# richardshuai/ExPecto

Hardware: AMD Instinct MI355X
Metric: variants/sec (200 windows × 2002 feats) at 1/2/4/8 MI355X; HBM GB/s vs peak (higher is better)
Workload: dtype fp32 in/out (f16x3: power-of-2-scaled 2-way fp16 split = 22-bit operands, 3 MFMA products, fp32 accumulate; bf16x6 recompute on fp16 overflow)

## Files before the change

### expecto_amd/csrc/beluga.hip

```cpp
#include <hip/hip_runtime.h>

#include <algorithm>
#include <array>
#include <cstdint>
#include <cstdlib>
#include <cstring>
#include <map>
#include <memory>
#include <mutex>
#include <tuple>
#include <string>
#include <vector>

#include "beluga_knobs.h"
#include "common.h"
#include "event_pairs.h"
#include "gemm_kernel.h"
#include "seg_plan.h"

namespace expecto {

static_assert(kStrandFwd == EXPECTO_STRAND_FWD && kStrandRc == EXPECTO_STRAND_RC && kStrandBoth == EXPECTO_STRAND_BOTH &&
              EXPECTO_EINVAL == -1, "seg_plan.h restates the strand modes and the refusal code");
constexpr int kNFeat = 2002;
// ... 475 lines not shown

__global__ __launch_bounds__(64) void slab_macs(const unsigned* __restrict__ mask, int tiles, double per_bit,
                                                double* __restrict__ acc) {
  int bits = 0;
  for (int i = threadIdx.x; i < tiles; i += 64) bits += __popc(mask[i]);
  for (int o = 32; o > 0; o >>= 1) bits += __shfl_down(bits, o);
  if (threadIdx.x == 0) atomicAdd(acc, bits * per_bit);
}

__global__ __launch_bounds__(256) void pair_patch_apply(const float* __restrict__ d6, float* __restrict__ act6, int nv,
                                                        int v0, const int* __restrict__ var_pos, int row16) {
  const int m = blockIdx.x;
  const int r6 = delta_rows(pair_pos(var_pos, m, nv, v0)).r[6];
  const floatx4* src = reinterpret_cast<const floatx4*>(d6) + (long long)m * kDW[6] * row16;
  floatx4* dst = reinterpret_cast<floatx4*>(act6) + ((long long)m * 106 + r6) * row16;
  for (int k = threadIdx.x; k < kDW[6] * row16; k += blockDim.x) dst[k] = src[k];
}

constexpr int kSegTab = 20;
constexpr int kW4u = 19, kA4u = 26;
struct SegDims {
  int L, T1, P1, T3, T4, S5, T5, T6;
};

__global__ void seg_delta_table(const int* __restrict__ var_pos, int e0, int ns, SegStrands ss, SegDims g, int n_ph,
                                int4 ph, int* __restrict__ tab) {
  const int m = blockIdx.x * blockDim.x + threadIdx.x;
  if (m >= ns) return;
  const int e = e0 + m;
  int q = min(max(var_pos[e >= ss.n_seg ? e - ss.n_seg : e], 0), g.L - 1);
  if (e >= ss.rc_ent) q = g.L - 1 - q;
  int* t = tab + m * kSegTab;
  const int r1 = clampi(q - 7, 0, g.T1 - kDW[1]);
  const int r2 = clampi(floor4(r1 - 7), 0, g.P1 - kDW[2]);
  const int r3 = clampi(r2 - 7, 0, g.T3 - kDW[3]);
  const int r4 = clampi(r3 - 7, 0, g.T4 - kW4u);
  t[0] = q;
  t[1] = r1;
  t[2] = r2;
  t[3] = r3;
  t[4] = r4;
  for (int i = 0; i < n_ph; ++i) {
    const int p = i == 0 ? ph.x : i == 1 ? ph.y : i == 2 ? ph.z : ph.w;
    const int r4p = clampi(floor4(r4 - p), 0, g.S5 - kDW[4]);
    const int r5 = clampi(r4p - 7, 0, g.T5 - kDW[5]);
    t[5 + i] = r4p;
// ... 163 lines not shown
  const int q = o >> 2, p = q & 3, off6 = (q - p) >> 2;
  const int pi = p == 0 ? ph_idx.x : p == 1 ? ph_idx.y : p == 2 ? ph_idx.z : ph_idx.w;
  const int r6 = tab[(win_seg[w] + sd * ss.n_seg - ent_base) * kSegTab + 13 + pi];
  const int lo = max(r6 - off6, 0), hi = min(r6 + kDW[6] - off6, 106);
  if (lo >= hi) return;
  unsigned bits = 0;
  for (int ks = lo * 640 / slab_k; ks <= (hi * 640 - 1) / slab_k; ++ks) bits |= 1u << ks;
  atomicOr(mask + m / tile_rows, bits);
}

__global__ void copy_rows(const float* __restrict__ src, float* __restrict__ dst, const int* __restrict__ widx,
                          const int* __restrict__ win_row, int n_win, long long rc_rows) {
  const int v = widx[blockIdx.x];
  const int sd = v >= n_win ? 1 : 0, w = v - sd * n_win;
  const long long r = (sd * rc_rows + (win_row ? win_row[w] : w)) * kNFeat;
  for (int i = threadIdx.x; i < kNFeat; i += blockDim.x) dst[r + i] = src[r + i];
}

__global__ void pair_rows(long long* __restrict__ c_rows, int M, int nv, int v0, long long strand_stride) {
  const int m = blockIdx.x * blockDim.x + threadIdx.x;
  if (m < M) c_rows[m] = (long long)(m / nv) * strand_stride + v0 + m % nv;
}

constexpr int kFkK = 16000;
constexpr int kFkKb = kFkK / GBK;
constexpr int kFkSlabs = 2;
constexpr int kFkTailK = kFc1In - 4 * kFkK;
constexpr int kFkKbTotal = 9 * kFkKb + kFkTailK / GBK;
constexpr long long kFkKTotal = 9LL * kFkK + kFkTailK;
constexpr int kFkSeq[9] = {3, 2, 3, 1, 0, 1, 3, 2, 3};
constexpr int kFkBlk[9] = {0, 1, 1, 2, 3, 3, 2, 3, 3};
constexpr int kFkRole[4][4] = {{0, 1, 3, 4}, {1, 2, 4, 5}, {3, 4, 6, 7}, {4, 5, 7, 8}};
constexpr int kFkW[9][4] = {{1, 0, 0, 0}, {1, 1, 0, 0}, {0, -1, 0, 0}, {1, 0, 1, 0}, {1, 1, 1, 1},
                            {0, -1, 0, -1}, {0, 0, -1, 0}, {0, 0, -1, -1}, {0, 0, 0, 1}};
constexpr int kFkParts = 4 * kFkSlabs + 1;

__global__ void fk_weights(const float* __restrict__ w1, long long rows, float* __restrict__ wk) {
  const long long i = (long long)blockIdx.x * blockDim.x + threadIdx.x;
  if (i >= rows * kFkKTotal) return;
  const long long n = i / kFkKTotal;
  const int k = (int)(i - n * kFkKTotal);
  const float* wr = w1 + n * kFc1In;
  if (k >= 9 * kFkK) {
    wk[i] = wr[4 * kFkK + (k - 9 * kFkK)];
    return;
  }
  const int g = k / kFkK, kk = k - g * kFkK;
  double s = 0.0;
#pragma unroll
  for (int q = 0; q < 4; ++q)
    if (kFkW[g][q]) s += kFkW[g][q] * (double)wr[q * kFkK + kk];
  wk[i] = (float)s;
}

__global__ __launch_bounds__(320) void fk_seq_h2(const float* __restrict__ x, int T, int s, const int* __restrict__ tab,
// ... 1306 lines not shown
    else
      fc2_reduce1<<<dim3((unsigned)(((long long)nb * kNFeat + 255) / 256)), dim3(256), 0, st>>>(
          h->part2, h->fc2_splits, (long long)nb * kHidLd, nb, h->fc2b, a.col_scale, c_rows, y);
    if ((rc = check_launch("fc2_reduce"))) return rc;
  }
  return EXPECTO_OK;
}

int run_fc(expecto_beluga* h, const float* act, const long long* a_rows, int nb, float* y, hipStream_t st,
           const long long* c_rows = nullptr, const unsigned* ks_mask = nullptr, double slab_frac = 1.0,
           long long part_rows = 0) {
  int rc;
  if ((rc = run_fc1(h, act, a_rows, nb, h->h1, st, ks_mask, slab_frac, part_rows))) return rc;
  return run_fc2(h, h->h1, nb, y, st, c_rows);
}

int count_desc_macs(expecto_beluga* h, const unsigned* mask, int tiles, double per_tile, hipStream_t st);

bool fk_use(const expecto_beluga* h) {
  return h->fk_on && h->fkw && g_precision == EXPECTO_PRECISION_F16X3 && h->fk_role < 4;
}
bool fk_use_seg(const expecto_beluga* h) { return h->fk_on && h->fkw && g_precision == EXPECTO_PRECISION_F16X3; }

int fk_cap(const expecto_beluga* h) { return std::max(h->max_batch, h->fk_slice); }
constexpr int kGresPerBatch = 3;

int fk_tables(expecto_beluga* h) {
  if (h->fk_grows) return EXPECTO_OK;
  const size_t mb = h->max_batch, tiles = (mb + 255) / 256, cap = fk_cap(h);
  float *a = nullptr, *b = nullptr, *c = nullptr, *d = nullptr;
  int rc;
  if ((rc = dalloc(h, &a, 2 * 9 * cap)) || (rc = dalloc(h, &b, 2 * mb)) || (rc = dalloc(h, &c, kFkParts * cap)) ||
      (rc = dalloc(h, &d, kFkParts * tiles)))
    return rc;
  h->fk_grows = reinterpret_cast<long long*>(a);
  h->fk_wrows = reinterpret_cast<long long*>(b);
  h->fk_prow = reinterpret_cast<int*>(c);
  h->fk_mask = reinterpret_cast<unsigned*>(d);
  return EXPECTO_OK;
}

int fk_seg_buffers(expecto_beluga* h) {
  if (h->fk_part) return EXPECTO_OK;
  const size_t cap = fk_cap(h);
  float *a = nullptr, *b = nullptr;
  int rc;
  if ((rc = dalloc(h, &h->fk_part, (size_t)kFkParts * cap * kHidLd)) || (rc = dalloc(h, &h->fk_h1, act_alloc(cap * kHidLd))) ||
// ... 20 lines not shown
    if ((rc = b.reserve(((size_t)rows + 16) * 640, h->bytes))) break;
  return rc;
}

int fk_sequences(expecto_beluga* h, const float* x, long long blocks, int T, int s, const int* tab, int n_ph,
                 hipStream_t st, const int* gres = nullptr, int set = 0) {
  int rc;
  if ((rc = fk_seq_alloc(h, blocks * s, set))) return rc;
  const DevBuf<float>* out = set ? h->fk_aseq : h->fk_seq;
  Timer lt(h, 7, st);
  const long long nblk = blocks * 7;
  EXPECTO_REQUIRE(nblk > 0 && nblk < (1LL << 31), "FC1 sequence grid");
  fk_seq_h2<<<dim3((unsigned)nblk), dim3(320), 0, st>>>(x, T, s, tab, n_ph, gres, out[0], out[1], out[2], h->ovf);
  return check_launch("fk_seq_h2");
}

struct FkProducts {
  const long long* g_rows;
  int off[9];
  int cnt[9];
  int lay[9];
};

int fk_reduce(expecto_beluga* h, const float* part, const int* prow, int n, float* h1, hipStream_t st) {
  Timer lt(h, 7, st);
  const long long count4 = (long long)n * (kHidLd / 4);
  fk_reduce_h2<<<dim3((unsigned)((count4 + 255) / 256)), dim3(256), 0, st>>>(part, prow, count4, h->fc1b, h1, h->fk_cs,
                                                                           exp2i(h->sx[6]), h->ovf);
  return check_launch("fk_reduce_h2");
}

constexpr int kFcNarrowNb = 7;
static_assert(kHidLd % (16 * kFcNarrowNb) == 0 && kHidLd % FCW_BN == 0, "FC1 N tiles");
bool fc1_narrow(const expecto_beluga* h, long long mtt) {
  if (h->fc1_narrow >= 0) return h->fc1_narrow != 0;
  if (!h->narrow_scope) return false;
  const long long cus = h->cus > 0 ? h->cus : 256;
  return mtt * (kHidLd / (16 * kFcNarrowNb)) <= cus;
}

static_assert(kHidLd % (16 * FCS_NB) == 0 &&
                  (kNFeat + 16 * FCS_NB - 1) / (16 * FCS_NB) * 16 * FCS_NB <= (kNFeat + GBN - 1) / GBN * GBN,
              "skinny FC tiles");
bool fc_skinny(const expecto_beluga* h, long long rows) {
  return h->fc_skinny && rows <= 32 && (h->fc1_narrow >= 0 ? h->fc1_narrow != 0 : h->narrow_scope);
}

int fk_fc1(expecto_beluga* h, const float* x, const DevBuf<float>* seq, const FkProducts& pr, const long long* w_rows, int n,
           const int* prow, float* h1, hipStream_t st, const unsigned* mask = nullptr, int tiles = 0,
           float* part = nullptr, long long part_cap = 0) {
  if (!part) {
    part = h->part;
    part_cap = (long long)std::max(h->fc_splits, kFkParts) * h->max_batch;
  }
  FcGroup G{};
  G.kb_total = kFkKbTotal;
  G.n_tiles = (kHidLd + FCW_BN - 1) / FCW_BN;
  G.n_store = kHidLd;
  G.ldc = kHidLd;
  const char* wb = reinterpret_cast<const char*>(h->fkw);
  long long row = 0;
  long long blk = 0;
  int mslot = 0;
  double macs = 0.0;
  auto add = [&](const float* A, const long long* ar, long long aoff, int kb0, int nk, int M, int lay) {
    FcDesc& d = G.d[G.n];
    d.A = A;
    d.a_rows = ar;
    d.a_off = aoff;
    d.Bp = wb + (long long)kb0 * 128;
    d.C = part + row * kHidLd;
    d.mask = mask ? mask + (size_t)mslot * tiles : nullptr;
    ++mslot;
    d.M = M;
    d.m_tiles = (M + X6P_BM - 1) / X6P_BM;
    d.nk = nk;
    d.blk0 = (int)blk;
    blk += (long long)d.m_tiles * G.n_tiles;
    row += lay;
    macs += (double)M * kFc1Out * nk * GBK;
    ++G.n;
  };
  for (int g = 0; g < 9; ++g) {
    const int lay = pr.lay[g] ? pr.lay[g] : pr.cnt[g];
    for (int s = 0; lay > 0 && s < kFkSlabs; ++s) {
      if (pr.cnt[g] > 0)
        add(kFkSeq[g] ? seq[kFkSeq[g] - 1].p : x, pr.g_rows + pr.off[g], 25LL * kFkBlk[g] * 640 + (long long)s * kFkK / kFkSlabs,
            g * kFkKb + s * kFkKb / kFkSlabs, kFkKb / kFkSlabs, pr.cnt[g], lay);
      else {
        row += lay;
        ++mslot;
      }
    }
  }
  add(x, w_rows, 100LL * 640, 9 * kFkKb, kFkTailK / GBK, n, n);
  EXPECTO_REQUIRE(G.n <= FCK_MAX && blk < (1LL << 31), "Karatsuba FC1 descriptors");
  EXPECTO_REQUIRE(row <= part_cap, "Karatsuba FC1 partial rows");
  {
    Timer lt(h, 6, st);
    if (h->profiling) {
      if (!mask) {
        h->macs[h->timer_base + 6] += macs;
      } else {
        for (int i = 0; i < G.n; ++i) {
          const FcDesc& d = G.d[i];
          int rc = count_desc_macs(h, d.mask, d.m_tiles, (double)d.M / d.m_tiles * kFc1Out * d.nk * GBK, st);
          if (rc) return rc;
        }
      }
    }
    G.rr = mask ? 0 : 1;
    const long long mtt = blk / G.n_tiles;
    const bool narrow = !mask && fc1_narrow(h, mtt);
    if (narrow) {
      G.n_tiles = kHidLd / (16 * kFcNarrowNb);
      for (int i = 0; i < G.n; ++i) G.d[i].blk0 = G.d[i].blk0 / (kHidLd / FCW_BN) * G.n_tiles;
    }
    const long long grid = G.rr ? (mtt + 7) / 8 * 8 * G.n_tiles : mtt * G.n_tiles;
    if (narrow)
      beluga_fc_h3k_narrow<<<dim3((unsigned)grid), dim3(512), 0, st>>>(G);
// ... 202 lines not shown
  return run_conv(c.h, l, c.h->DA, dnext, (long long)ck.ns * nbk, arows, w, w, pool, c.sa);
}
int seg_st_wait(const SegCall& c, hipEvent_t e) {
  if (c.sa != c.st) EXPECTO_HIP_CHECK(hipStreamWaitEvent(c.st, e, 0));
  return EXPECTO_OK;
}

int seg_rows(const SegCall& c, const SegChunk& ck, const int* widx, int w0, int n, long long* a_rows,
             long long* c_rows) {
  seg_a_rows<<<dim3((n + 255) / 256), dim3(256), 0, c.st>>>(c.h->win_seg_d, c.h->win_off_d, c.win_row_d, widx, w0, n,
                                                             ck.s0, c.pl.ss, c.pl.g.L, c.pl.n_ph, c.phi, c.pl.g.T6,
                                                             a_rows, c_rows);
  return check_launch("seg_a_rows");
}

int seg_fc2(const SegCall& c, const float* h1, int n, float* y, const long long* c_rows) {
  int rc;
  for (int r0 = 0; r0 < n; r0 += c.h->max_batch)
    if ((rc = run_fc2(c.h, h1 + (long long)r0 * kHidLd, std::min(c.h->max_batch, n - r0), y, c.st, c_rows + r0)))
      return rc;
  return EXPECTO_OK;
}

int seg_alt_conv6(const SegCall& c, const SegChunk& ck) {
  int rc;
  if ((rc = seg_st_wait(c, c.h->pev[13]))) return rc;
  seg_alt_blocks<<<dim3(kAltRows6, (unsigned)ck.nb), dim3(64), 0, c.st>>>(c.h->P, c.h->D0, c.pl.n_ph, c.pl.g.T6,
                                                                           c.h->seg_tab, 640 * c.eb / 16, c.h->Q);
  return check_launch("seg_alt_blocks");
}

int seg_copy_tail(const SegCall& c, const SegChunk& ck) {
  if (!c.pr) return EXPECTO_OK;
  const std::vector<int>& cw = c.pl.copy_w;
  const int ic0 = (int)(std::lower_bound(cw.begin(), cw.end(), ck.w0) - cw.begin());
  const int ic1 = (int)(std::lower_bound(cw.begin(), cw.end(), ck.w0 + ck.nw) - cw.begin());
  if (ic1 <= ic0) return EXPECTO_OK;
  copy_rows<<<dim3(ic1 - ic0), dim3(256), 0, c.st>>>(c.y, c.pr->y_alt, c.h->copy_w_d + ic0, c.win_row_d, c.pl.ss.n_win,
                                                      c.pl.ss.rc_rows);
  return check_launch("copy_rows");
}

int seg_trunk(const SegCall& c, const SegChunk& ck, PQSwap& pq) {
  expecto_beluga* h = c.h;
  const SegPairs* pr = c.pr;
  const SegGeo& g = c.pl.g;
  const hipStream_t st = c.st, sa = c.sa;
  const int s0 = ck.s0, ns = ck.ns, n_ph = c.pl.n_ph;
  const long long nb = ck.nb;
  int rc;
  if (pr && (rc = stream_order(st, sa, h->pev[0]))) return rc;
// ... 111 lines not shown
    t.pa.cnt[gq] = cnt;
    t.pa.lay[gq] = prd.cnt[gq];
    for (int sb = 0; prd.cnt[gq] > 0 && sb < kFkSlabs; ++sb) {
      t.md.g[t.md.n] = gq;
      t.md.s[t.md.n] = sb;
      t.md.off[t.md.n] = prd.off[gq];
      t.md.cnt[t.md.n] = cnt;
      ++t.md.n;
    }
  }
  t.md.nw = (int)sl.nw_pre;
  for (size_t i = 0; i < sl.nw_pre; ++i) {
    const FkWin& w = ws[sl.i0 + i];
    t.winfo.push_back(w.blk);
    t.winfo.push_back(w.off6);
    if (pl.v_is_alt(w.w)) {
      t.aperm.push_back(w.w);
      t.aprow.insert(t.aprow.end(), prow.begin() + (long long)i * kFkParts, prow.begin() + (long long)(i + 1) * kFkParts);
    }
  }
  return t;
}

int seg_fc_karatsuba(const SegCall& c, const SegChunk& ck) {
  expecto_beluga* h = c.h;
  const SegPlan& pl = c.pl;
  const hipStream_t st = c.st;
  const int T6 = pl.g.T6, n_ph = pl.n_ph;
  const long long nb = ck.nb, cap = pl.fk_cap;
  const std::vector<FkWin>& ws = pl.fk_ref[ck.ci];
  const int* perm = h->fc_perm_d + ck.w0;
  int rc;
  const std::vector<int> gres = pl.fk_gres(ck.ci);
  EXPECTO_REQUIRE(nb <= kGresPerBatch * (long long)h->max_batch, "conv6 blocks of a chunk exceed fk_gres");
  if ((rc = stage_copies(h, {{h->fk_gres, gres.data(), gres.size() * sizeof(int)}}, st)) || (rc = fk_tables(h)) ||
      (rc = fk_seg_buffers(h)) || (rc = fk_sequences(h, h->P, nb, T6, T6, nullptr, n_ph, st, h->fk_gres)))
    return rc;
  bool alt_ready = false;
  FkSlice sl{};
  for (size_t i0 = 0; i0 < ws.size(); i0 = sl.i1) {
    const char* refusal = pl.fk_slice(ck.ci, i0, sl);
    EXPECTO_REQUIRE(!refusal, refusal);
    const int fn = (int)(sl.i1 - i0);
    std::vector<long long> grows;
    std::vector<int> prow, rgrp, ginfo;
    FkProducts prd{h->fk_grows, {}, {}, {}};
    fk_slice_tables(ws, (int)i0, (int)sl.i1, T6, grows, prd, prow, &rgrp, &ginfo);
    if ((rc = stage_copies(h, {{h->fk_grows, grows.data(), grows.size() * sizeof(long long)},
                               {h->fk_prow, prow.data(), prow.size() * sizeof(int)}}, st)) ||
        (rc = seg_rows(c, ck, perm + i0, 0, fn, h->fk_arows, h->fk_crows)) ||
        (rc = fk_fc1(h, h->P, h->fk_seq, prd, h->fk_arows, fn, h->fk_prow, h->fk_h1, st, nullptr, 0, h->fk_part,
                     kFkParts * cap)) ||
        (rc = seg_fc2(c, h->fk_h1, fn, c.y, h->fk_crows)))
      return rc;
    if (sl.n_ag == 0) continue;
    const FkAltTables t = fk_alt_tables(pl, ws, sl, prd, rgrp, prow);
    const int na = (int)t.aperm.size();
    const int tiles = (int)(cap / 256 + 1);
    if ((rc = stage_copies(h, {{h->fk_rgrp, rgrp.data(), rgrp.size() * sizeof(int)},
                               {h->fk_ginfo, ginfo.data(), ginfo.size() * sizeof(int)},
                               {h->fk_winfo, t.winfo.data(), t.winfo.size() * sizeof(int)},
                               {h->fk_aperm, t.aperm.data(), t.aperm.size() * sizeof(int)},
                               {h->fk_aprow, t.aprow.data(), t.aprow.size() * sizeof(int)}}, st)))
      return rc;
    if (!alt_ready) {
      if ((rc = seg_alt_conv6(c, ck))) return rc;
      DeltaScope ds(h);
      if ((rc = fk_sequences(h, h->Q, nb, T6, T6, h->seg_tab, n_ph, st, h->fk_gres, 1))) return rc;
      alt_ready = true;
    }
    EXPECTO_HIP_CHECK(hipMemsetAsync(h->fk_smask, 0, (size_t)(t.md.n + 1) * tiles * sizeof(unsigned), st));
    int rows_max = t.md.nw;
    for (int i = 0; i < t.md.n; ++i) rows_max = std::max(rows_max, t.md.cnt[i]);
    if (rows_max > 0) {
      fk_seg_mask<<<dim3((rows_max + 255) / 256, t.md.n + 1), dim3(256), 0, st>>>(
          t.md, h->fk_rgrp, h->fk_ginfo, h->fk_winfo, h->seg_tab, n_ph, make_int4(0, 0, 0, 0), tiles, h->fk_smask);
      if ((rc = check_launch("fk_seg_mask"))) return rc;
    }
    DeltaScope ds(h);
    if ((rc = fk_fc1(h, h->Q, h->fk_aseq, t.pa, h->fk_arows, (int)sl.nw_pre, nullptr, h->fk_h1, st, h->fk_smask, tiles,
                     h->fk_part, kFkParts * cap)) ||
        (na > 0 && ((rc = fk_reduce(h, h->fk_part, h->fk_aprow, na, h->fk_h1, st)) ||
                    (rc = seg_rows(c, ck, h->fk_aperm, 0, na, h->fk_arows, h->fk_crows)) ||
                    (rc = seg_fc2(c, h->fk_h1, na, c.pr->y_alt, h->fk_crows)))))
      return rc;
  }
  return seg_copy_tail(c, ck);
}

int seg_fc_direct(const SegCall& c, const SegChunk& ck) {
  expecto_beluga* h = c.h;
// ... 47 lines not shown
    DeltaScope ds(h);
    if (gather2) {
      float* h1a = h1_rows(h, h->fc2_rows);
      if ((rc = run_fc1(h, h->Q, h->a_rows, na, h1a, st, mask, frac, fn)) ||
          (rc = run_fc2(h, h1a, na, pr->y_alt, st, acrow)))
        return rc;
    } else if ((rc = run_fc(h, h->Q, h->a_rows, na, pr->y_alt, st, h->c_rows, mask, frac, fn))) {
      return rc;
    }
  }
  if ((rc = flush2())) return rc;
  return seg_copy_tail(c, ck);
}

int forward_segments(expecto_beluga* h, const uint8_t* codes, int n_seg, int L, long long code_stride, int mode,
                     const int* win_seg, const int* win_off, const int* win_row, int n_win, float* y,
                     hipStream_t st, const SegPairs* pr = nullptr) {
  g_precision = h->precision;
  g_conv_ea = h->conv_ea;
  SegPlan pl;
  const char* refusal = nullptr;
  if (seg_plan({n_seg, L, mode, win_seg, win_off, win_row, n_win, pr ? pr->var_pos : nullptr,
                pr ? pr->strand_stride : n_win, h->max_batch, p_floats(h->max_batch) - 16 * 640,
                q_floats(h->max_batch) - 16 * 640, h->seg_merge_strands, h->seg_chunk_windows, fk_use_seg(h), fk_cap(h)},
               pl, &refusal)) {
    set_error(refusal);
    return EXPECTO_EINVAL;
  }
  int rc;
  if (pr && (rc = ensure_delta(h))) return rc;
  const size_t nw = (size_t)n_win;
  if ((rc = h->win_seg_d.reserve(nw, h->bytes)) || (rc = h->win_off_d.reserve(nw, h->bytes)) ||
      (rc = h->win_row_d.reserve(nw, h->bytes)) || (rc = h->alt_w_d.reserve(2 * nw, h->bytes)) ||
      (rc = h->copy_w_d.reserve(2 * nw, h->bytes)) || (rc = h->fc_perm_d.reserve(4 * nw, h->bytes)) ||
      (pr && (rc = h->seg_var_d.reserve((size_t)n_seg, h->bytes))))
    return rc;
  std::vector<HostCopy> copies;
  if (pr) {
    copies.push_back({h->seg_var_d, pr->var_pos, n_seg * sizeof(int)});
    copies.push_back({h->alt_w_d, pl.alt_w.data(), pl.alt_w.size() * sizeof(int)});
    copies.push_back({h->copy_w_d, pl.copy_w.data(), pl.copy_w.size() * sizeof(int)});
  }
  if (win_row) copies.push_back({h->win_row_d, win_row, n_win * sizeof(int)});
  copies.push_back({h->win_seg_d, win_seg, n_win * sizeof(int)});
  copies.push_back({h->win_off_d, win_off, n_win * sizeof(int)});
  if (!pl.fc_perm.empty()) copies.push_back({h->fc_perm_d, pl.fc_perm.data(), pl.fc_perm.size() * sizeof(int)});
  if ((rc = stage_copies(h, copies, st))) return rc;
// ... 683 lines not shown
```

### expecto_amd/csrc/beluga_knobs.h

```cpp
#pragma once

#include <algorithm>
#include <cstdlib>
#include <limits>

namespace expecto {

constexpr int kFc1KBlocks = 2120;
constexpr int kFc2KBlocks = 63;
constexpr int kFc2SplitsDefault = 7;
constexpr int kFcSplitsDefault = 8;

struct BelugaKnobs {
  bool overlap = true;
  int fc_splits = kFcSplitsDefault;
  int fc2_splits = kFc2SplitsDefault;
  int fc2_rows_env = 0;
  double fc1_m_order_mb = 80.0;
  int fc1_order = 3;
  int fc1_m_group = 8;
  bool fc_wide = true;
  int conv_tile = 0;
  bool conv_ea = true;
  bool fc_skinny = true;
  int fc1_narrow = -1;
  int conv_narrow = -1;
  int seg_chunk_windows = 0;
  bool seg_merge_strands = true;
  bool pool_one_pass = true;
  bool pool_fused = true;
  bool fuse_conv1 = true;
  bool kmer_on = true;
  bool kmer_quad = true;
  double kmer_max_bytes = std::numeric_limits<double>::infinity();
  bool fk_on = true;
  int fk_role = 4;
  int fk_slice = 24576;
  bool onehot_as_codes = true;
};

struct BelugaKnob {
  const char* name;
  bool BelugaKnobs::*b;
  int BelugaKnobs::*i;
  double BelugaKnobs::*d;
  int floor;
  bool (*ok)(int);
  const char* refusal;
};

namespace knob_detail {
using K = BelugaKnobs;
constexpr int kAny = std::numeric_limits<int>::min();
constexpr BelugaKnob flag(const char* n, bool K::*f) { return {n, f, nullptr, nullptr, kAny, nullptr, nullptr}; }
constexpr BelugaKnob num(const char* n, int K::*f, int floor = kAny, bool (*ok)(int) = nullptr, const char* why = nullptr) {
  return {n, nullptr, f, nullptr, floor, ok, why};
}
constexpr BelugaKnob real(const char* n, double K::*f) { return {n, nullptr, nullptr, f, kAny, nullptr, nullptr}; }
inline bool fc1_splits_ok(int v) { return v >= 1 && v <= 32 && kFc1KBlocks % v == 0; }
inline bool fc2_splits_ok(int v) { return v >= 1 && kFc2KBlocks % v == 0; }
// ... 16 lines not shown
    knob_detail::flag("EXPECTO_POOL_ONE_PASS", &BelugaKnobs::pool_one_pass),
    knob_detail::flag("EXPECTO_POOL_FUSED", &BelugaKnobs::pool_fused),
    knob_detail::flag("EXPECTO_FUSE_CONV1", &BelugaKnobs::fuse_conv1),
    knob_detail::flag("EXPECTO_CONV2_TABLE", &BelugaKnobs::kmer_on),
    knob_detail::flag("EXPECTO_KMER_QUAD", &BelugaKnobs::kmer_quad),
    knob_detail::real("EXPECTO_KMER_MAX_BYTES", &BelugaKnobs::kmer_max_bytes),
    knob_detail::flag("EXPECTO_ONEHOT_CODES", &BelugaKnobs::onehot_as_codes),
    knob_detail::flag("EXPECTO_FC1_KARATSUBA", &BelugaKnobs::fk_on),
    knob_detail::num("EXPECTO_FC1K_SLICE", &BelugaKnobs::fk_slice, 1),
    knob_detail::num("EXPECTO_FC1_ROLE", &BelugaKnobs::fk_role, knob_detail::kAny, knob_detail::role_ok,
                     "EXPECTO_FC1_ROLE must be 0..4"),
    knob_detail::num("EXPECTO_SEG_CHUNK_WINDOWS", &BelugaKnobs::seg_chunk_windows),
    knob_detail::flag("EXPECTO_SEG_MERGE_STRANDS", &BelugaKnobs::seg_merge_strands),
    knob_detail::num("EXPECTO_CONV_NARROW", &BelugaKnobs::conv_narrow, knob_detail::kAny, knob_detail::tri_ok,
                     "EXPECTO_CONV_NARROW must be -1 (auto), 0 or 1"),
    knob_detail::num("EXPECTO_FC1_NARROW", &BelugaKnobs::fc1_narrow, knob_detail::kAny, knob_detail::tri_ok,
                     "EXPECTO_FC1_NARROW must be -1 (auto), 0 or 1"),
    knob_detail::flag("EXPECTO_CONV_EA", &BelugaKnobs::conv_ea),
    knob_detail::flag("EXPECTO_FC_SKINNY", &BelugaKnobs::fc_skinny),
    knob_detail::num("EXPECTO_CONV_TILE", &BelugaKnobs::conv_tile, knob_detail::kAny, knob_detail::conv_tile_ok,
                     "EXPECTO_CONV_TILE must be 0 (auto), 256 or 384"),
};

template <class Getenv>
const char* beluga_knobs_parse(BelugaKnobs& k, Getenv&& get) {
  for (const BelugaKnob& s : kBelugaKnobs) {
    const char* e = get(s.name);
    if (!e) continue;
    if (s.b) {
      k.*s.b = atoi(e) != 0;
    } else if (s.d) {
      k.*s.d = atof(e);
    } else {
      const int v = std::max(s.floor, atoi(e));
      if (s.ok && !s.ok(v)) return s.refusal;
      k.*s.i = v;
    }
  }
  return nullptr;
}

}
```

### expecto_amd/csrc/gemm_kernel.h

```cpp
#pragma once
#include <hip/hip_runtime.h>

#include <type_traits>

namespace expecto {

typedef float floatx4 __attribute__((ext_vector_type(4)));
typedef float floatx16 __attribute__((ext_vector_type(16)));

constexpr int GBN = 160;
constexpr int GBK = 32;
constexpr int GTN = GBN / 32;

enum { EPI_RELU = 0, EPI_RELU_POOL4 = 1, EPI_SIGMOID = 2, EPI_PARTIAL = 3, EPI_POOL_PH02 = 4 };

struct GemmArgs {
  const float* A;
  long long lda;
  long long M;
  const float* B;
  long long ldb;
  int kper;
  int taps;
  int n_tiles;
// ... 1186 lines not shown
      bf16x8 a[3], b[3];
      a[0] = *(const bf16x8*)(base + arow);
      a[1] = *(const bf16x8*)(base + arow + G::APLANE);
      b[0] = *(const bf16x8*)(base + brow);
      b[1] = *(const bf16x8*)(base + brow + G::BPLANE);
      acc = planes_mfma<2>(acc, a, b);
    }
    stage_end_wait();
    __builtin_amdgcn_s_barrier();
    asm volatile("" ::: "memory");
  }
  asm volatile("s_waitcnt vmcnt(0)" ::: "memory");
  if (!live) return;
  const int n = n0 + nb * 16 + fr;
  if (n >= p.n_store) return;
  float* cp = p.C + (long long)ks * p.split_stride + n;
#pragma unroll
  for (int j = 0; j < 4; ++j) {
    const long long m = mb * 16 + 4 * fq + j;
    if (m < p.M) cp[m * p.ldc] = acc[j];
  }
}

constexpr int FCK_MAX = 24;
struct FcDesc {
  const float* A;
  const long long* a_rows;
  long long a_off;
  const char* Bp;
  float* C;
  const unsigned* mask;
  int M, m_tiles, nk, blk0;
};
struct FcGroup {
  FcDesc d[FCK_MAX];
  int n, kb_total, n_tiles, n_store;
  long long ldc;
  int rr;
};

template <int TM, int NB, int NS = 2>
__device__ __forceinline__ void fc_h3k_body(const FcGroup& g, char* smem) {
  const unsigned nblk = gridDim.x, bid = blockIdx.x;
  int k = 0, mt, nt;
  if (g.rr) {
    const int slot = (int)(bid >> 3);
    const int T = (slot / g.n_tiles) * 8 + (int)(bid & 7u);
// ... 958 lines not shown
```

### expecto_amd/csrc/seg_plan.h

```cpp
#pragma once

#include <algorithm>
#include <cstddef>
#include <map>
#include <tuple>
#include <utility>
#include <vector>

namespace expecto {

constexpr int kLen = 2000;
enum { kStrandFwd = 0, kStrandRc = 1, kStrandBoth = 2 };

struct SegStrands {
  int n_seg, rc_ent, n_win, rc_win;
  long long rc_rows;
};

struct SegGeo {
  int L, T1, S1, P1, T3, T4, S5, T5, T6;
  size_t p_rows_floats, q_rows_floats;
};

inline SegGeo seg_geo(int L, int n_ph) {
// ... 9 lines not shown
  g.T6 = g.T5 - 7;
  const size_t p_conv1 = (size_t)g.S1 * 320, p_conv3 = (size_t)((g.T3 + 3) & ~3) * 480, p_pool2 = (size_t)n_ph * g.S5 * 480,
               p_conv6 = (size_t)n_ph * g.T6 * 640;
  const size_t q_pool1 = (size_t)g.P1 * 320, q_conv4 = (size_t)g.T4 * 480, q_conv5 = (size_t)n_ph * g.T5 * 640;
  g.p_rows_floats = std::max(std::max(p_conv1, p_conv3), std::max(p_pool2, p_conv6));
  g.q_rows_floats = std::max(q_pool1, std::max(q_conv4, q_conv5));
  return g;
}

struct FkWin {
  int w, blk, off6;
};
inline int fk_role_of(int off6) { return (off6 / 25) & 3; }
inline int fk_group_of(int off6) { return off6 - 25 * fk_role_of(off6); }
inline FkWin fk_win(int w, int seg, int off, bool rc, int L, int n_ph, const int* ph_idx) {
  const int o = rc ? L - kLen - off : off;
  const int q = o >> 2, p = q & 3;
  return {w, seg * n_ph + ph_idx[p], (q - p) >> 2};
}
inline bool fk_same_group(const FkWin& a, const FkWin& b) {
  return a.blk == b.blk && fk_group_of(a.off6) == fk_group_of(b.off6);
}

struct SegPlanIn {
  int n_seg, L, mode;
  const int *win_seg, *win_off, *win_row;
  int n_win;
  const int* var_pos;
  long long rc_rows;
  int max_batch;
  size_t p_cap, q_cap;
  bool merge_strands;
  int chunk_windows;
  bool fk;
  long long fk_cap;
};

struct FkSlice {
  size_t i0, i1, nw_pre;
  int n_ag;
};

struct SegPlan {
  int present[4], n_ph, ph[4], ph_idx[4];
  SegGeo g;
  int seg_cap;
  SegStrands ss;
  int n_ent, n_vw;
  int blk_per_seg;
  bool pairs;
  std::vector<int> first, vfirst;
  std::vector<char> is_alt;
  std::vector<int> alt_w, copy_w;
  std::vector<std::pair<int, int>> chunks;
  std::vector<int> fc_perm;
  bool fkm;
  std::vector<std::vector<FkWin>> fk_ref, fk_alt;
  long long fk_cap;

  int vw_w(int v) const { return v >= ss.n_win ? v - ss.n_win : v; }
  bool v_is_alt(int v) const { return is_alt[vw_w(v)] != 0; }

  std::vector<int> fk_gres(size_t ci) const {
    std::vector<int> gres((size_t)(chunks[ci].second - chunks[ci].first) * n_ph, -2);
    for (const FkWin& w : fk_ref[ci]) {
      const int r = fk_group_of(w.off6) % 100;
      int& e = gres[(size_t)w.blk];
      e = e == -2 ? r : (e == r ? r : -1);
    }
    return gres;
  }

  const char* fk_slice(size_t ci, size_t i0, FkSlice& s) const {
    const std::vector<FkWin>& ws = fk_ref[ci];
    size_t i1 = i0;
    while (i1 < ws.size()) {
      size_t j = i1 + 1;
      while (j < ws.size() && fk_same_group(ws[j], ws[i1])) ++j;
      if (j - i0 > (size_t)fk_cap && i1 > i0) break;
      i1 = j;
    }
    if (i1 - i0 > (size_t)fk_cap) return "a Karatsuba FC1 window group exceeds the FC1 slice";
    s = {i0, i1, 0, 0};
    const bool has_alt = pairs && !fk_alt[ci].empty();
    for (size_t i = i0; has_alt && i < i1; ++i) {
      bool galt = false;
      size_t j = i;
      for (; j < i1 && fk_same_group(ws[j], ws[i]); ++j) galt |= v_is_alt(ws[j].w);
      if (!galt) break;
      ++s.n_ag;
      s.nw_pre = j - i0;
      i = j - 1;
    }
    return nullptr;
  }
};

inline int seg_plan(const SegPlanIn& in, SegPlan& p, const char** err) {
#define SEG_PLAN_REQUIRE(cond, msg) \
  do {                              \
    if (!(cond)) {                  \
      *err = msg;                   \
      return -1;                    \
    }                               \
  } while (0)
  const int n_seg = in.n_seg, L = in.L, mode = in.mode, n_win = in.n_win;
  const int *win_seg = in.win_seg, *win_off = in.win_off;
  SEG_PLAN_REQUIRE(L >= kLen && L % 4 == 0, "segment length must be >= 2000 and a multiple of 4");
  for (int i = 0; i < 4; ++i) p.present[i] = p.ph[i] = p.ph_idx[i] = 0;
  for (int w = 0; w < n_win; ++w) {
    SEG_PLAN_REQUIRE(win_seg[w] >= 0 && win_seg[w] < n_seg, "window segment out of range");
    SEG_PLAN_REQUIRE(w == 0 || win_seg[w] >= win_seg[w - 1], "windows must be sorted by segment");
    const int o = win_off[w];
    SEG_PLAN_REQUIRE(o >= 0 && o % 4 == 0 && o + kLen <= L, "window offset must be 4-aligned inside the segment");
    if (mode != kStrandRc) p.present[(o >> 2) & 3] = 1;
    if (mode != kStrandFwd) p.present[((L - kLen - o) >> 2) & 3] = 1;
  }
// ... 26 lines not shown
    for (int w = 0; w < n_win; ++w) {
      const int q = in.var_pos[win_seg[w]];
      p.is_alt[w] = win_off[w] <= q && q < win_off[w] + kLen;
    }
    for (int v = 0; v < n_vw; ++v) (p.v_is_alt(v) ? p.alt_w : p.copy_w).push_back(v);
  }
  if (in.win_row)
    for (int w = 0; w < n_win; ++w)
      SEG_PLAN_REQUIRE(in.win_row[w] >= 0 && in.win_row[w] < n_win, "window row out of range");
#undef SEG_PLAN_REQUIRE
  p.blk_per_seg = p.pairs ? std::max(n_ph, 1) : 0;
  p.chunks.clear();
  for (int e0 = 0; e0 < n_ent;) {
    int e1 = e0 + 1;
    while (e1 < n_ent && (e1 != n_seg || in.merge_strands) && e1 - e0 < p.seg_cap &&
           (long long)(e1 + 1 - e0) * p.blk_per_seg <= in.max_batch &&
           (in.chunk_windows <= 0 || p.vfirst[e1 + 1] - p.vfirst[e0] <= in.chunk_windows))
      ++e1;
    p.chunks.push_back({e0, e1});
    e0 = e1;
  }
  p.fkm = in.fk && !(p.pairs && 3 * p.alt_w.size() > (size_t)n_vw);
  p.fk_cap = in.fk_cap;
  p.fc_perm.clear();
  p.fk_ref.clear();
  p.fk_alt.clear();
  if (p.pairs && !p.fkm) {
    p.fc_perm.resize((size_t)n_vw);
    auto pos_of = [&](int v) {
      const int w = p.vw_w(v), q = in.var_pos[win_seg[w]] - win_off[w];
      return v >= p.ss.rc_win ? kLen - 1 - q : q;
    };
    for (const auto& c : p.chunks) {
      const int w0 = p.vfirst[c.first], w1 = p.vfirst[c.second];
      int k = w0;
      std::vector<int> a;
      for (int v = w0; v < w1; ++v)
        if (p.v_is_alt(v)) a.push_back(v);
      std::stable_sort(a.begin(), a.end(), [&](int x, int y) { return pos_of(x) < pos_of(y); });
      for (int v : a) p.fc_perm[k++] = v;
      for (int v = w0; v < w1; ++v)
        if (!p.v_is_alt(v)) p.fc_perm[k++] = v;
    }
  }
  if (p.fkm) {
    p.fc_perm.assign((size_t)4 * n_win, 0);
// ... 48 lines not shown
```

Baseline: 1521.

## Fold alt-allele Karatsuba FC1 products into the ref FC1 launch with sparse rows

```diff
diff --git a/expecto_amd/csrc/beluga.hip b/expecto_amd/csrc/beluga.hip
--- a/expecto_amd/csrc/beluga.hip
+++ b/expecto_amd/csrc/beluga.hip
@@ -521,6 +521,9 @@
 struct SegDims {
   int L, T1, P1, T3, T4, S5, T5, T6;
 };
+static_assert(kSegW[1] == kDW[1] && kSegW[2] == kDW[2] && kSegW[3] == kDW[3] && kSegW[4] == kW4u && kSegW[5] == kDW[4] &&
+                  kSegW[6] == kDW[5] && kSegW6 == kDW[6],
+              "seg_plan.h seg_r6 restates seg_delta_table's run widths");
 
 __global__ void seg_delta_table(const int* __restrict__ var_pos, int e0, int ns, SegStrands ss, SegDims g, int n_ph,
                                 int4 ph, int* __restrict__ tab) {
@@ -730,15 +733,10 @@
   if (m < M) c_rows[m] = (long long)(m / nv) * strand_stride + v0 + m % nv;
 }
 
-constexpr int kFkK = 16000;
 constexpr int kFkKb = kFkK / GBK;
-constexpr int kFkSlabs = 2;
 constexpr int kFkTailK = kFc1In - 4 * kFkK;
 constexpr int kFkKbTotal = 9 * kFkKb + kFkTailK / GBK;
 constexpr long long kFkKTotal = 9LL * kFkK + kFkTailK;
-constexpr int kFkSeq[9] = {3, 2, 3, 1, 0, 1, 3, 2, 3};
-constexpr int kFkBlk[9] = {0, 1, 1, 2, 3, 3, 2, 3, 3};
-constexpr int kFkRole[4][4] = {{0, 1, 3, 4}, {1, 2, 4, 5}, {3, 4, 6, 7}, {4, 5, 7, 8}};
 constexpr int kFkW[9][4] = {{1, 0, 0, 0}, {1, 1, 0, 0}, {0, -1, 0, 0}, {1, 0, 1, 0}, {1, 1, 1, 1},
                             {0, -1, 0, -1}, {0, 0, -1, 0}, {0, 0, -1, -1}, {0, 0, 0, 1}};
 constexpr int kFkParts = 4 * kFkSlabs + 1;
@@ -2091,7 +2089,10 @@
 }
 bool fk_use_seg(const expecto_beluga* h) { return h->fk_on && h->fkw && g_precision == EXPECTO_PRECISION_F16X3; }
 
-int fk_cap(const expecto_beluga* h) { return std::max(h->max_batch, h->fk_slice); }
+int fk_cap(const expecto_beluga* h) {
+  const long long dflt = std::min<long long>((long long)kFkSlicePerBatch * h->max_batch, 1LL << 30);
+  return std::max(h->max_batch, h->fk_slice ? h->fk_slice : (int)dflt);
+}
 constexpr int kGresPerBatch = 3;
 
 int fk_tables(expecto_beluga* h) {
@@ -2158,6 +2159,16 @@
   int lay[9];
 };
 
+struct FkAltRows {
+  const float* x;
+  const DevBuf<float>* seq;
+  const long long* g_rows;
+  int off[9][kFkSlabs], cnt[9][kFkSlabs];
+  const long long* w_rows;
+  int n_tail;
+  long long row0;
+};
+
 int fk_reduce(expecto_beluga* h, const float* part, const int* prow, int n, float* h1, hipStream_t st) {
   Timer lt(h, 7, st);
   const long long count4 = (long long)n * (kHidLd / 4);
@@ -2184,7 +2195,7 @@
 
 int fk_fc1(expecto_beluga* h, const float* x, const DevBuf<float>* seq, const FkProducts& pr, const long long* w_rows, int n,
            const int* prow, float* h1, hipStream_t st, const unsigned* mask = nullptr, int tiles = 0,
-           float* part = nullptr, long long part_cap = 0) {
+           float* part = nullptr, long long part_cap = 0, const FkAltRows* alt = nullptr) {
   if (!part) {
     part = h->part;
     part_cap = (long long)std::max(h->fc_splits, kFkParts) * h->max_batch;
@@ -2199,13 +2210,17 @@
   long long blk = 0;
   int mslot = 0;
   double macs = 0.0;
-  auto add = [&](const float* A, const long long* ar, long long aoff, int kb0, int nk, int M, int lay) {
+  auto add = [&](const float* A, const long long* ar, long long aoff, int kb0, int nk, int M, long long crow) {
+    if (G.n >= FCK_MAX) {
+      ++G.n;
+      return;
+    }
     FcDesc& d = G.d[G.n];
     d.A = A;
     d.a_rows = ar;
     d.a_off = aoff;
     d.Bp = wb + (long long)kb0 * 128;
-    d.C = part + row * kHidLd;
+    d.C = part + crow * kHidLd;
     d.mask = mask ? mask + (size_t)mslot * tiles : nullptr;
     ++mslot;
     d.M = M;
@@ -2213,7 +2228,6 @@
     d.nk = nk;
     d.blk0 = (int)blk;
     blk += (long long)d.m_tiles * G.n_tiles;
-    row += lay;
     macs += (double)M * kFc1Out * nk * GBK;
     ++G.n;
   };
@@ -2222,16 +2236,31 @@
     for (int s = 0; lay > 0 && s < kFkSlabs; ++s) {
       if (pr.cnt[g] > 0)
         add(kFkSeq[g] ? seq[kFkSeq[g] - 1].p : x, pr.g_rows + pr.off[g], 25LL * kFkBlk[g] * 640 + (long long)s * kFkK / kFkSlabs,
-            g * kFkKb + s * kFkKb / kFkSlabs, kFkKb / kFkSlabs, pr.cnt[g], lay);
-      else {
-        row += lay;
+            g * kFkKb + s * kFkKb / kFkSlabs, kFkKb / kFkSlabs, pr.cnt[g], row);
+      else
         ++mslot;
-      }
-    }
-  }
-  add(x, w_rows, 100LL * 640, 9 * kFkKb, kFkTailK / GBK, n, n);
+      row += lay;
+    }
+  }
+  const long long tail_row = row;
+  row += n;
+  long long arow = alt ? alt->row0 : row;
+  EXPECTO_REQUIRE(!(alt && mask) && arow >= row, "Karatsuba FC1 alt rows");
+  for (int g = 0; alt && g < 9; ++g)
+    for (int s = 0; s < kFkSlabs; ++s) {
+      if (alt->cnt[g][s] <= 0) continue;
+      add(kFkSeq[g] ? alt->seq[kFkSeq[g] - 1].p : alt->x, alt->g_rows + alt->off[g][s],
+          25LL * kFkBlk[g] * 640 + (long long)s * kFkK / kFkSlabs, g * kFkKb + s * kFkKb / kFkSlabs, kFkKb / kFkSlabs,
+          alt->cnt[g][s], arow);
+      arow += alt->cnt[g][s];
+    }
+  add(x, w_rows, 100LL * 640, 9 * kFkKb, kFkTailK / GBK, n, tail_row);
+  if (alt && alt->n_tail > 0) {
+    add(alt->x, alt->w_rows, 100LL * 640, 9 * kFkKb, kFkTailK / GBK, alt->n_tail, arow);
+    arow += alt->n_tail;
+  }
   EXPECTO_REQUIRE(G.n <= FCK_MAX && blk < (1LL << 31), "Karatsuba FC1 descriptors");
-  EXPECTO_REQUIRE(row <= part_cap, "Karatsuba FC1 partial rows");
+  EXPECTO_REQUIRE(arow <= part_cap, "Karatsuba FC1 partial rows");
   {
     Timer lt(h, 6, st);
     if (h->profiling) {
@@ -2480,11 +2509,12 @@
   return EXPECTO_OK;
 }
 
-int seg_alt_conv6(const SegCall& c, const SegChunk& ck) {
+int seg_alt_conv6(const SegCall& c, const SegChunk& ck, bool on_sa = false) {
   int rc;
-  if ((rc = seg_st_wait(c, c.h->pev[13]))) return rc;
-  seg_alt_blocks<<<dim3(kAltRows6, (unsigned)ck.nb), dim3(64), 0, c.st>>>(c.h->P, c.h->D0, c.pl.n_ph, c.pl.g.T6,
-                                                                           c.h->seg_tab, 640 * c.eb / 16, c.h->Q);
+  const hipStream_t s = on_sa ? c.sa : c.st;
+  if ((rc = s == c.st ? seg_st_wait(c, c.h->pev[13]) : stream_order(c.st, s, c.h->pev[14]))) return rc;
+  seg_alt_blocks<<<dim3(kAltRows6, (unsigned)ck.nb), dim3(64), 0, s>>>(c.h->P, c.h->D0, c.pl.n_ph, c.pl.g.T6,
+                                                                        c.h->seg_tab, 640 * c.eb / 16, c.h->Q);
   return check_launch("seg_alt_blocks");
 }
 
@@ -2642,6 +2672,77 @@
   return t;
 }
 
+int seg_alt_sequences(const SegCall& c, const SegChunk& ck, bool on_sa) {
+  expecto_beluga* h = c.h;
+  on_sa = on_sa && c.sa != c.st;
+  int rc;
+  if ((rc = seg_alt_conv6(c, ck, on_sa))) return rc;
+  DeltaScope ds(h);
+  if ((rc = fk_sequences(h, h->Q, ck.nb, c.pl.g.T6, c.pl.g.T6, h->seg_tab, c.pl.n_ph, on_sa ? c.sa : c.st, h->fk_gres, 1)))
+    return rc;
+  if (on_sa) EXPECTO_HIP_CHECK(hipEventRecord(h->pev[15], c.sa));
+  return EXPECTO_OK;
+}
+
+struct FkAltRowTables {
+  FkAltRows ar;
+  size_t w_off;
+  std::vector<int> perm;
+  long long rows;
+};
+FkAltRowTables fk_alt_row_tables(const std::vector<FkWin>& ws, const FkSlice& sl, const FkAltPlan& ap, int T6,
+                                 long long row0, std::vector<long long>& grows, std::vector<int>& prow) {
+  FkAltRowTables t{};
+  t.ar.row0 = row0;
+  std::vector<long long> gst;
+  for (size_t i = sl.i0; i < sl.i0 + sl.nw_pre; ++i)
+    if (i == sl.i0 || !fk_same_group(ws[i], ws[i - 1]))
+      gst.push_back(((long long)ws[i].blk * T6 + fk_group_of(ws[i].off6)) * 640);
+  long long base[9][kFkSlabs] = {}, row = row0;
+  for (int g = 0; g < 9; ++g)
+    for (int sb = 0; sb < kFkSlabs; ++sb) {
+      const std::vector<int>& l = ap.grp[g][sb];
+      t.ar.off[g][sb] = (int)grows.size();
+      t.ar.cnt[g][sb] = (int)l.size();
+      base[g][sb] = row;
+      row += (long long)l.size();
+      for (int k : l) grows.push_back(gst[(size_t)k]);
+    }
+  t.w_off = grows.size();
+  t.ar.n_tail = (int)ap.tail.size();
+  for (int i : ap.tail) grows.push_back(((long long)ws[sl.i0 + i].blk * T6 + ws[sl.i0 + i].off6) * 640);
+  const long long tail_base = row;
+  t.rows = row + (long long)ap.tail.size() - row0;
+  const int fn = (int)(sl.i1 - sl.i0);
+  for (int i = 0; i < fn; ++i) t.perm.push_back(ws[sl.i0 + i].w);
+  auto pos_in = [](const std::vector<int>& l, int v) {
+    const auto it = std::lower_bound(l.begin(), l.end(), v);
+    return it != l.end() && *it == v ? (int)(it - l.begin()) : -1;
+  };
+  int k = -1;
+  size_t next = 0;
+  for (size_t i = 0; i < sl.nw_pre && next < ap.win.size(); ++i) {
+    if (i == 0 || !fk_same_group(ws[sl.i0 + i], ws[sl.i0 + i - 1])) ++k;
+    if ((int)i != ap.win[next]) continue;
+    ++next;
+    const FkWin& w = ws[sl.i0 + i];
+    t.perm.push_back(w.w);
+    const size_t p0 = prow.size();
+    prow.resize(p0 + kFkParts);
+    for (int j = 0; j < kFkParts; ++j) prow[p0 + j] = prow[i * kFkParts + j];
+    for (int j = 0; j < 4; ++j) {
+      const int g = kFkRole[fk_role_of(w.off6)][j];
+      for (int sb = 0; sb < kFkSlabs; ++sb) {
+        const int at = pos_in(ap.grp[g][sb], k);
+        if (at >= 0) prow[p0 + kFkSlabs * j + sb] = (int)(base[g][sb] + at);
+      }
+    }
+    const int at = pos_in(ap.tail, (int)i);
+    if (at >= 0) prow[p0 + kFkParts - 1] = (int)(tail_base + at);
+  }
+  return t;
+}
+
 int seg_fc_karatsuba(const SegCall& c, const SegChunk& ck) {
   expecto_beluga* h = c.h;
   const SegPlan& pl = c.pl;
@@ -2654,9 +2755,16 @@
   const std::vector<int> gres = pl.fk_gres(ck.ci);
   EXPECTO_REQUIRE(nb <= kGresPerBatch * (long long)h->max_batch, "conv6 blocks of a chunk exceed fk_gres");
   if ((rc = stage_copies(h, {{h->fk_gres, gres.data(), gres.size() * sizeof(int)}}, st)) || (rc = fk_tables(h)) ||
-      (rc = fk_seg_buffers(h)) || (rc = fk_sequences(h, h->P, nb, T6, T6, nullptr, n_ph, st, h->fk_gres)))
+      (rc = fk_seg_buffers(h)))
     return rc;
   bool alt_ready = false;
+  const bool alt_early = c.pr && !h->fk_alt_inplace && !pl.fk_alt[ck.ci].empty();
+  if (alt_early) {
+    if ((rc = seg_alt_sequences(c, ck, true))) return rc;
+    alt_ready = true;
+  }
+  if ((rc = fk_sequences(h, h->P, nb, T6, T6, nullptr, n_ph, st, h->fk_gres))) return rc;
+  if (alt_early && (rc = seg_st_wait(c, h->pev[15]))) return rc;
   FkSlice sl{};
   for (size_t i0 = 0; i0 < ws.size(); i0 = sl.i1) {
     const char* refusal = pl.fk_slice(ck.ci, i0, sl);
@@ -2666,6 +2774,33 @@
     std::vector<int> prow, rgrp, ginfo;
     FkProducts prd{h->fk_grows, {}, {}, {}};
     fk_slice_tables(ws, (int)i0, (int)sl.i1, T6, grows, prd, prow, &rgrp, &ginfo);
+    if (sl.n_ag > 0 && !h->fk_alt_inplace) {
+      const FkAltPlan ap = pl.fk_alt_plan(ck.ci, sl);
+      const int na = (int)ap.win.size();
+      long long ref_rows = fn, alt_lists = (long long)ap.tail.size();
+      for (int g = 0; g < 9; ++g) {
+        ref_rows += (long long)kFkSlabs * prd.cnt[g];
+        for (int sb = 0; sb < kFkSlabs; ++sb) alt_lists += (long long)ap.grp[g][sb].size();
+      }
+      if (fn + na <= cap && ref_rows + alt_lists <= kFkParts * cap && (long long)grows.size() + alt_lists <= 9 * cap) {
+        FkAltRowTables t = fk_alt_row_tables(ws, sl, ap, T6, ref_rows, grows, prow);
+        t.ar.x = h->Q;
+        t.ar.seq = h->fk_aseq;
+        t.ar.g_rows = h->fk_grows;
+        t.ar.w_rows = h->fk_grows + t.w_off;
+        if ((rc = stage_copies(h, {{h->fk_grows, grows.data(), grows.size() * sizeof(long long)},
+                                   {h->fk_prow, prow.data(), prow.size() * sizeof(int)},
+                                   {h->fk_aperm, t.perm.data(), t.perm.size() * sizeof(int)}}, st)) ||
+            (rc = seg_rows(c, ck, h->fk_aperm, 0, fn + na, h->fk_arows, h->fk_crows)) ||
+            (rc = fk_fc1(h, h->P, h->fk_seq, prd, h->fk_arows, fn, nullptr, h->fk_h1, st, nullptr, 0, h->fk_part,
+                         kFkParts * cap, &t.ar)) ||
+            (rc = fk_reduce(h, h->fk_part, h->fk_prow, fn + na, h->fk_h1, st)) ||
+            (rc = seg_fc2(c, h->fk_h1, fn, c.y, h->fk_crows)) ||
+            (na > 0 && (rc = seg_fc2(c, h->fk_h1 + (long long)fn * kHidLd, na, c.pr->y_alt, h->fk_crows + fn))))
+          return rc;
+        continue;
+      }
+    }
     if ((rc = stage_copies(h, {{h->fk_grows, grows.data(), grows.size() * sizeof(long long)},
                                {h->fk_prow, prow.data(), prow.size() * sizeof(int)}}, st)) ||
         (rc = seg_rows(c, ck, perm + i0, 0, fn, h->fk_arows, h->fk_crows)) ||
@@ -2684,9 +2819,7 @@
                                {h->fk_aprow, t.aprow.data(), t.aprow.size() * sizeof(int)}}, st)))
       return rc;
     if (!alt_ready) {
-      if ((rc = seg_alt_conv6(c, ck))) return rc;
-      DeltaScope ds(h);
-      if ((rc = fk_sequences(h, h->Q, nb, T6, T6, h->seg_tab, n_ph, st, h->fk_gres, 1))) return rc;
+      if ((rc = seg_alt_sequences(c, ck, false))) return rc;
       alt_ready = true;
     }
     EXPECTO_HIP_CHECK(hipMemsetAsync(h->fk_smask, 0, (size_t)(t.md.n + 1) * tiles * sizeof(unsigned), st));
@@ -2780,7 +2913,8 @@
   const char* refusal = nullptr;
   if (seg_plan({n_seg, L, mode, win_seg, win_off, win_row, n_win, pr ? pr->var_pos : nullptr,
                 pr ? pr->strand_stride : n_win, h->max_batch, p_floats(h->max_batch) - 16 * 640,
-                q_floats(h->max_batch) - 16 * 640, h->seg_merge_strands, h->seg_chunk_windows, fk_use_seg(h), fk_cap(h)},
+                q_floats(h->max_batch) - 16 * 640, h->seg_merge_strands, h->seg_chunk_windows, fk_use_seg(h), fk_cap(h),
+                h->fk_alt_inplace},
                pl, &refusal)) {
     set_error(refusal);
     return EXPECTO_EINVAL;
diff --git a/expecto_amd/csrc/beluga_knobs.h b/expecto_amd/csrc/beluga_knobs.h
--- a/expecto_amd/csrc/beluga_knobs.h
+++ b/expecto_amd/csrc/beluga_knobs.h
@@ -10,6 +10,8 @@
 constexpr int kFc2KBlocks = 63;
 constexpr int kFc2SplitsDefault = 7;
 constexpr int kFcSplitsDefault = 8;
+
+constexpr int kFkSlicePerBatch = 5;
 
 struct BelugaKnobs {
   bool overlap = true;
@@ -35,7 +37,8 @@
   double kmer_max_bytes = std::numeric_limits<double>::infinity();
   bool fk_on = true;
   int fk_role = 4;
-  int fk_slice = 24576;
+  int fk_slice = 0;
+  bool fk_alt_inplace = false;
   bool onehot_as_codes = true;
 };
 
@@ -98,6 +101,10 @@
                      "EXPECTO_CONV_TILE must be 0 (auto), 256 or 384"),
 };
 
+inline constexpr BelugaKnob kBelugaSwitches[] = {
+    knob_detail::flag("EXPECTO_FC1K_ALT_INPLACE", &BelugaKnobs::fk_alt_inplace),
+};
+
 template <class Getenv>
 const char* beluga_knobs_parse(BelugaKnobs& k, Getenv&& get) {
   for (const BelugaKnob& s : kBelugaKnobs) {
@@ -113,6 +120,8 @@
       k.*s.i = v;
     }
   }
+  for (const BelugaKnob& s : kBelugaSwitches)
+    if (const char* e = get(s.name)) k.*s.b = atoi(e) != 0;
   return nullptr;
 }
 
diff --git a/expecto_amd/csrc/gemm_kernel.h b/expecto_amd/csrc/gemm_kernel.h
--- a/expecto_amd/csrc/gemm_kernel.h
+++ b/expecto_amd/csrc/gemm_kernel.h
@@ -1232,7 +1232,7 @@
   }
 }
 
-constexpr int FCK_MAX = 24;
+constexpr int FCK_MAX = 40;
 struct FcDesc {
   const float* A;
   const long long* a_rows;
diff --git a/expecto_amd/csrc/seg_plan.h b/expecto_amd/csrc/seg_plan.h
--- a/expecto_amd/csrc/seg_plan.h
+++ b/expecto_amd/csrc/seg_plan.h
@@ -55,6 +55,39 @@
   return a.blk == b.blk && fk_group_of(a.off6) == fk_group_of(b.off6);
 }
 
+constexpr int kFkK = 16000;
+constexpr int kFkSlabs = 2;
+constexpr int kFkSeq[9] = {3, 2, 3, 1, 0, 1, 3, 2, 3};
+constexpr int kFkBlk[9] = {0, 1, 1, 2, 3, 3, 2, 3, 3};
+constexpr int kFkRole[4][4] = {{0, 1, 3, 4}, {1, 2, 4, 5}, {3, 4, 6, 7}, {4, 5, 7, 8}};
+
+constexpr int kSegW[7] = {0, 8, 5, 12, 19, 6, 13};
+constexpr int kSegW6 = 20;
+inline int seg_floor4(int v) { return v >= 0 ? v >> 2 : -((3 - v) >> 2); }
+inline int seg_clamp(int v, int lo, int hi) { return v < lo ? lo : (v > hi ? hi : v); }
+inline int seg_r6(const SegGeo& g, int q, int p) {
+  const int r1 = seg_clamp(q - 7, 0, g.T1 - kSegW[1]);
+  const int r2 = seg_clamp(seg_floor4(r1 - 7), 0, g.P1 - kSegW[2]);
+  const int r3 = seg_clamp(r2 - 7, 0, g.T3 - kSegW[3]);
+  const int r4 = seg_clamp(r3 - 7, 0, g.T4 - kSegW[4]);
+  const int r4p = seg_clamp(seg_floor4(r4 - p), 0, g.S5 - kSegW[5]);
+  const int r5 = seg_clamp(r4p - 7, 0, g.T5 - kSegW[6]);
+  return seg_clamp(r5 - 7, 0, g.T6 - kSegW6);
+}
+
+inline bool fk_reach(int G, int g, int s, int r6) {
+  const int base = G + 25 * kFkBlk[g], per = kFkK / kFkSlabs;
+  const int i0 = base + (s * per) / 640, i1 = base + ((s + 1) * per - 1) / 640;
+  const int sq = kFkSeq[g], nl = sq == 0 ? 1 : sq == 3 ? 4 : 2, lag1 = sq == 2 ? 50 : 25;
+  bool hit = false;
+  for (int l = 0; l < nl; ++l) {
+    const int lag = l == 0 ? 0 : (nl == 2 ? lag1 : 25 * l);
+    hit |= i0 + lag < r6 + kSegW6 && i1 + lag >= r6;
+  }
+  return hit;
+}
+inline bool fk_reach_tail(int off6, int r6) { return off6 + 100 < r6 + kSegW6 && off6 + 105 >= r6; }
+
 struct SegPlanIn {
   int n_seg, L, mode;
   const int *win_seg, *win_off, *win_row;
@@ -67,11 +100,17 @@
   int chunk_windows;
   bool fk;
   long long fk_cap;
+  bool alt_inplace = false;
 };
 
 struct FkSlice {
   size_t i0, i1, nw_pre;
   int n_ag;
+};
+
+struct FkAltPlan {
+  std::vector<int> grp[9][kFkSlabs];
+  std::vector<int> win, tail;
 };
 
 struct SegPlan {
@@ -90,6 +129,8 @@
   bool fkm;
   std::vector<std::vector<FkWin>> fk_ref, fk_alt;
   long long fk_cap;
+  bool alt_inplace;
+  std::vector<int> r6;
 
   int vw_w(int v) const { return v >= ss.n_win ? v - ss.n_win : v; }
   bool v_is_alt(int v) const { return is_alt[vw_w(v)] != 0; }
@@ -106,11 +147,14 @@
 
   const char* fk_slice(size_t ci, size_t i0, FkSlice& s) const {
     const std::vector<FkWin>& ws = fk_ref[ci];
-    size_t i1 = i0;
+    const bool twice = pairs && !alt_inplace && !fk_alt[ci].empty();
+    size_t i1 = i0, rows = 0;
     while (i1 < ws.size()) {
-      size_t j = i1 + 1;
-      while (j < ws.size() && fk_same_group(ws[j], ws[i1])) ++j;
-      if (j - i0 > (size_t)fk_cap && i1 > i0) break;
+      size_t j = i1, n = 0;
+      do n += twice && v_is_alt(ws[j].w) ? 2 : 1;
+      while (++j < ws.size() && fk_same_group(ws[j], ws[i1]));
+      if (rows + n > (size_t)fk_cap && i1 > i0) break;
+      rows += n;
       i1 = j;
     }
     if (i1 - i0 > (size_t)fk_cap) return "a Karatsuba FC1 window group exceeds the FC1 slice";
@@ -126,6 +170,28 @@
       i = j - 1;
     }
     return nullptr;
+  }
+
+  FkAltPlan fk_alt_plan(size_t ci, const FkSlice& s) const {
+    const std::vector<FkWin>& ws = fk_ref[ci];
+    FkAltPlan a;
+    int k = -1;
+    for (size_t i = s.i0; i < s.i0 + s.nw_pre; ++i) {
+      if (i == s.i0 || !fk_same_group(ws[i], ws[i - 1])) ++k;
+      const FkWin& w = ws[i];
+      if (!v_is_alt(w.w)) continue;
+      const int r = r6[(size_t)chunks[ci].first * n_ph + w.blk];
+      a.win.push_back((int)(i - s.i0));
+      if (fk_reach_tail(w.off6, r)) a.tail.push_back((int)(i - s.i0));
+      for (int j = 0; j < 4; ++j) {
+        const int g = kFkRole[fk_role_of(w.off6)][j];
+        for (int sb = 0; sb < kFkSlabs; ++sb) {
+          std::vector<int>& l = a.grp[g][sb];
+          if (fk_reach(fk_group_of(w.off6), g, sb, r) && (l.empty() || l.back() != k)) l.push_back(k);
+        }
+      }
+    }
+    return a;
   }
 };
 
@@ -198,6 +264,13 @@
   }
   p.fkm = in.fk && !(p.pairs && 3 * p.alt_w.size() > (size_t)n_vw);
   p.fk_cap = in.fk_cap;
+  p.alt_inplace = in.alt_inplace;
+  p.r6.clear();
+  if (p.pairs)
+    for (int e = 0; e < n_ent; ++e) {
+      const int q = in.var_pos[e >= n_seg ? e - n_seg : e];
+      for (int i = 0; i < n_ph; ++i) p.r6.push_back(seg_r6(p.g, e >= p.ss.rc_ent ? L - 1 - q : q, p.ph[i]));
+    }
   p.fc_perm.clear();
   p.fk_ref.clear();
   p.fk_alt.clear();
```

After: 1541 (median of 6 runs). +1.3%, better.
